# imaginateit/csm-train-pytorch

Measured on AMD Instinct MI355X. Metric: train tokens/sec (text+audio) CSM-1B bf16 seq2048, higher is better.
Workload: dtype bf16

## Files before the change

### csm-train-pytorch_amd/csm/engine.py

```python
from __future__ import annotations

from contextlib import contextmanager
from typing import Dict, List, Optional

import torch

from .hip import ops
from .sampling import (RowSampler, _is_number, check_filters, check_processors, check_row_processors,
                       check_sampling, names_processors)

BF16 = torch.bfloat16
F32 = torch.float32
import os as _os
FUSE_SWIGLU = _os.environ.get("CSM_FUSE_SWIGLU", "1") == "1"
FUSE_ROPE_BWD = _os.environ.get("CSM_FUSE_ROPE_BWD", "1") == "1"
FUSE_ROPE_FWD = _os.environ.get("CSM_FUSE_ROPE_FWD", "1") == "1"
PAIR_DX_DW = int(_os.environ.get("CSM_PAIR_DX_DW", "0"))
GROUP_ATTN_DW = _os.environ.get("CSM_GROUP_ATTN_DW", "1") == "1"
DEFER_ATTN_DW = int(_os.environ.get("CSM_DEFER_ATTN_DW", "3"))
DEFER_NORM_DW = _os.environ.get("CSM_DEFER_NORM_DW", "1") == "1"
ROWS_ON_HOST = _os.environ.get("CSM_ROWS_ON_HOST", "1") == "1"
EMB_KEYSORT = _os.environ.get("CSM_EMB_KEYSORT", "1") == "1"
DECODE_POS_HOST = _os.environ.get("CSM_DECODE_POS_HOST", "1") == "1"
LORA_FUSE = _os.environ.get("CSM_LORA_FUSE", "1") != "0"


def _refuse_stack(lo, where: str):
    if getattr(lo, "n_adapters", 1) > 1:
        raise ValueError(f"{where} takes one adapter set, and model.lora stacks {lo.n_adapters}: export one first "
                         "(state = model.lora.export(a), then LoRABank.add / generate_batch(adapters=[...]) / row_lora(model, state))")


def adapter_rows(adapter_ids, B: int, S: int, n_adapters: int, segment_lengths=None) -> torch.Tensor:
    ids = torch.as_tensor(adapter_ids).detach().to("cpu")
    if ids.is_floating_point() or ids.dtype == torch.bool:
        raise ValueError(f"adapter_ids must be integers, got {ids.dtype}")
    ids = ids.to(torch.int64)
    if segment_lengths is None:
        if tuple(ids.shape) != (B,):
            raise ValueError(f"adapter_ids must have shape [B={B}] (one adapter set per example), got {tuple(ids.shape)}")
        live = ids
        sel = ids.repeat_interleave(S)
    else:
        L = torch.as_tensor(segment_lengths).detach().to("cpu").to(torch.int64)
        if ids.dim() != 2 or tuple(ids.shape) != tuple(L.shape) or L.shape[0] != B:
            raise ValueError(f"adapter_ids of a packed batch must have the shape of segment_lengths {tuple(L.shape)} "
                             f"(one adapter set per segment), got {tuple(ids.shape)}")
        if bool((L < 0).any()) or bool((L.sum(1) > S).any()):
            raise ValueError("segment_lengths: negative, or more than a row holds")
        live = ids[L > 0]
        full_len = torch.cat([L, (S - L.sum(1))[:, None]], 1).reshape(-1)
        full_ids = torch.cat([ids, torch.full((B, 1), -1, dtype=torch.int64)], 1).reshape(-1)
        sel = torch.repeat_interleave(full_ids, full_len)
    if live.numel() and (int(live.min()) < -1 or int(live.max()) >= n_adapters):
        bad = live[(live < -1) | (live >= n_adapters)]
# ... 602 lines not shown
            ops.gemm(dl[0], ah[0], dxf[:, dd:2 * dd], None, False, False, batch=K - 1, sA=N * Vp, sB=dd * Vp, sC=dd)
            xf2 = dec["xf"].view(N, K * dd)
            if train_other:
                gah = m.block("audio_head.padded", True)
                ops.gemm(xf2[:, dd:2 * dd], dl[0], gah[0], gah[0] if acc["other"] else None, True, True, batch=K - 1, sA=dd,
                         sB=N * Vp, sC=dd * Vp, sR=dd * Vp)
            del dl
            dx0 = self.decoder.backward(dxf.view(N * K, dd), N, K, tr["decoder"], 1.0, on_layer_done=self.grad_hook,
                                        acc=acc["decoder"], sel=dec.get("sel"))
            dseq = torch.empty(N * K, d, dtype=BF16, device=dev)
            ops.linear_dx(dx0, m.block("projection.weight"), dseq)
            if train_other:
                ops.linear_dw(dx0, dec["seq"], m.block("projection.weight", True), accumulate=acc["other"])
            dec_pos0 = (dseq, dec["rows"], K)
            if self.grad_hook is not None:
                self.grad_hook("decoder", -1)

        dlog = torch.empty(M, Vp, dtype=BF16, device=dev)
        rows_loss = torch.empty(M, dtype=F32, device=dev)
        ops.ce_fwd_bwd(s["logits"], s["t0"], rows_loss, dlog, V, gscale * s["sw"] / s["n_sem"])
        dhid = torch.empty(M, d, dtype=BF16, device=dev)
        ops.linear_dx(dlog, m.block("codebook0_head.padded"), dhid)
        if train_other:
            ops.linear_dw(dlog, hidden, m.block("codebook0_head.padded", True), accumulate=acc["other"])
        del dlog
        if dec_pos0 is not None:
            ops.rows_add_bf16(dhid, dec_pos0[1], dec_pos0[0], dec_pos0[2])
        if self.grad_hook is not None:
            self.grad_hook("other", -1)

        dh0 = self.backbone.backward(dhid, B, S, tr["backbone"], 1.0, on_layer_done=self.grad_hook, acc=acc["backbone"], seg=s.get("seg"),
                                    sel=s.get("sel"))
        if train_embeddings:
            self._embedding_backward(s, dh0, dseq if (dec is not None and s["aw"] != 0.0) else None)
        if self.grad_hook is not None:
            self.grad_hook("embeddings", -1)

    def _embedding_backward(self, s, dh0, dseq):
        m, a = self.m, self.m.args
        dev = m.device
        K, V = a.audio_num_codebooks, a.audio_vocab_size
        TV = a.text_vocab_size
        n_rows = TV + K * V
        tk, mk = s["tk"], s["mk"]
        M = tk.shape[0]
        ck = ("embbwd", M, K, V, TV)
        c = self._consts.get(ck)
        if c is None:
            slot = torch.arange(K + 1, device=dev)
            c = self._consts[ck] = dict(off=torch.where(slot < K, TV + slot * V, torch.zeros_like(slot)),
                                        src=torch.arange(M, device=dev).unsqueeze(1).expand(M, K + 1).reshape(-1).contiguous())
        rows = torch.where(mk.bool(), tk + c["off"], torch.full_like(tk, n_rows)).reshape(-1)
        src = c["src"]
        n_src = M
        if dseq is not None:
            codes, N = s["dec"]["codes"], s["dec"]["N"]
            dk = ("embbwd_dec", M, N, K, V, TV)
            d = self._consts.get(dk)
            if d is None:
                d = self._consts[dk] = dict(off=TV + torch.arange(K - 1, device=dev) * V,
                                            src=(M + torch.arange(N, device=dev).unsqueeze(1) * K + torch.arange(1, K, device=dev)).reshape(-1))
            rows = torch.cat([rows, (codes[:, :K - 1] + d["off"]).reshape(-1)])
            src = torch.cat([src, d["src"]])
            n_src = M + N * K
        if n_src <= (1 << 20) and EMB_KEYSORT:
            key = torch.sort((rows << 20) | src).values
            rows_s, src_s = key >> 20, key & ((1 << 20) - 1)
        else:
            order = torch.argsort(rows, stable=True)
            rows_s, src_s = rows[order].contiguous(), src[order].contiguous()
        ops.embed_bwd_sorted(rows_s, src_s, dh0, dseq,
                             m.block("text_embeddings.weight", True), m.block("audio_embeddings.weight", True))

    @torch.no_grad()
    def hidden_states(self, tokens: torch.Tensor, masks: torch.Tensor) -> torch.Tensor:
        m, a = self.m, self.m.args
        B, S, K1 = tokens.shape
        M = B * S
        tk = tokens.reshape(M, K1).to(device=m.device, dtype=torch.int64).contiguous()
        mk = masks.reshape(M, K1).to(device=m.device, dtype=torch.uint8).contiguous()
        h0 = torch.empty(M, m.bb.embed_dim, dtype=BF16, device=m.device)
        self._need()
        ops.embed_fwd(tk, mk, m.block("text_embeddings.weight"), m.block("audio_embeddings.weight"), h0, a.audio_vocab_size)
        return self.backbone.forward(h0, B, S, False).view(B, S, -1)

    @torch.no_grad()
    def generate_frame(self, tokens, tokens_mask, input_pos, temperature, topk, noise=None, adapters=None, top_p=None,
                       min_p=None, repetition_penalty=None, repetition_window=None):
        m, a = self.m, self.m.args
        self._need()
        if int(input_pos[0, 0]) == 0:
            m._gen_adapters = list(adapters) if adapters is not None and any(x is not None for x in adapters) else None
        if not getattr(m, "use_kv_cache", True):
            if names_processors(temperature, topk, repetition_penalty=repetition_penalty, repetition_window=repetition_window):
                raise ValueError("the recompute path (use_kv_cache = False) has no repetition penalty and no per-codebook "
                                 "parameters: they need the KV-cache path")
            if top_p is not None or min_p is not None:
                raise ValueError("the recompute path (use_kv_cache = False) has no top_p / min_p: the filters need the KV-cache path")
            return self._generate_frame_recompute(tokens, tokens_mask, input_pos, temperature, topk, noise)
        dev = m.device
        K, V, Vp = a.audio_num_codebooks, a.audio_vocab_size, m.vocab_pad
        d, dd = m.bb.embed_dim, m.dc.embed_dim
        tokens, tokens_mask = tokens.to(dev), tokens_mask.to(dev)
        Bn, Sn, K1 = tokens.shape
        first = int(input_pos[0, 0]) == 0
# ... 688 lines not shown
```

### csm-train-pytorch_amd/csm/hip/__init__.py

```python
import ctypes as C
import os

_HERE = os.path.dirname(os.path.abspath(__file__))
LIB_PATH = os.environ.get("CSM_HIP_LIB") or os.path.join(_HERE, "libcsm_hip.so")


class CsmHipError(RuntimeError):
    pass


if not os.path.exists(LIB_PATH):
    raise ImportError(
        f"{LIB_PATH} is missing: build it with `python __graft_entry__.py build` (or `make -C csm-train-pytorch_amd/csrc`). "
        "The CSM MI355X path has no fallback implementation."
    )

lib = C.CDLL(LIB_PATH)

_p, _i, _f, _ll = C.c_void_p, C.c_int, C.c_float, C.c_longlong

_SIGS = {
    "csm_abi_version": ([], _i),
    "csm_last_error": ([], C.c_char_p),
    "csm_device_check": ([_i], _i),
# ... 5 lines not shown
    "csm_skinny_nt_bf16": ([_p, _p, _p, _i, _i, _i, _i, _i, _i, _f, _p], _i),
    "csm_skinny_nt_sel_bf16": ([_p, _p, _p, _p, _i, _i, _i, _i, _i, _i, _i, _f, _p], _i),
    "csm_gemm_bf16_dgrad_wgrad": ([_p, _p, _p, _p, _p, _i, _i, _i, _i, _i, _i, _i, _i, _i, _p, _i, _i, _f, _p], _i),
    "csm_gemm_bf16_two_wgrad": ([_p, _p, _p, _i, _i, _i, _i, _i, _p, _p, _p, _i, _i, _i, _i, _i, _i, _i, _f, _p], _i),
    "csm_gemm_bf16_multi_wgrad": ([_i, _p, _p, _p, _p, _p, _p, _p, _p, _i, _i, _f, _p], _i),
    "csm_set_gemm_variant": ([_i], _i),
    "csm_set_gemm256_persistent": ([_i], _i),
    "csm_get_gemm256_persistent": ([], _i),
    "csm_set_gemm_tuning": ([_i, _i], _i),
    "csm_gemm_last_kernel": ([], C.c_char_p),
    "csm_attn_bwd_workspace_bytes": ([_i, _i, _i], _ll),
    "csm_rmsnorm_fwd": ([_p, _p, _p, _p, _i, _i, _f, _p], _i),
    "csm_rmsnorm_bwd_blocks": ([], _i),
    "csm_rmsnorm_bwd": ([_p, _p, _p, _p, _p, _p, _p, _i, _i, _p], _i),
    "csm_colsum_bf16": ([_p, _i, _i, _p, _i, _p], _i),
    "csm_colsum_bf16_multi": ([_i, _p, _p, _i, _i, _i, _p], _i),
    "csm_dropout_bf16": ([_p, _i, _p, _i, _ll, _i, _f, C.c_ulonglong, _i, _p], _i),
    "csm_bias_add_bf16": ([_p, _i, _p, _ll, _i, _p], _i),
    "csm_colsum_rows_bf16": ([_p, _i, _ll, _i, _p, _i, _p], _i),
    "csm_rope": ([_p, _p, _p, _ll, _i, _i, _i, _i, _i, _p], _i),
    "csm_set_attn_variant": ([_i], _i),
    "csm_attn_last_dkv_kernel": ([], _i),
    "csm_attn64_set_debug": ([_p], _i),
    "csm_set_decode_tuning": ([_i, _i], _i),
    "csm_attn_fwd": ([_p, _p, _p, _i, _i, _i, _i, _i, _p], _i),
    "csm_attn_bwd": ([_p, _p, _p, _p, _p, _p, _i, _i, _i, _i, _i, _p], _i),
    "csm_attn_bwd_rope": ([_p, _p, _p, _p, _p, _p, _p, _i, _i, _i, _i, _i, _p], _i),
    "csm_attn_fwd_seg": ([_p, _p, _p, _p, _i, _i, _i, _i, _i, _p], _i),
    "csm_attn_bwd_seg": ([_p, _p, _p, _p, _p, _p, _p, _p, _i, _i, _i, _i, _i, _p], _i),
    "csm_swiglu_fwd": ([_p, _p, _ll, _i, _p], _i),
    "csm_swiglu_bwd": ([_p, _p, _p, _ll, _i, _p], _i),
    "csm_embed_fwd": ([_p, _p, _p, _p, _p, _ll, _i, _i, _i, _p], _i),
    "csm_embed_bwd_sorted": ([_p, _p, _ll, _p, _p, _ll, _p, _p, _ll, _ll, _i, _p], _i),
    "csm_rows_add_bf16": ([_p, _p, _p, _ll, _i, _i, _p], _i),
    "csm_rows_take_bf16": ([_p, _p, _p, _ll, _i, _p], _i),
    "csm_decoder_input_fwd": ([_p, _p, _p, _p, _p, _ll, _i, _i, _i, _p], _i),
    "csm_ce_fwd_bwd": ([_p, _p, _p, _p, _ll, _i, _i, _i, _f, _p], _i),
    "csm_reduce_sum_f32": ([_p, _ll, _f, _p, _p], _i),
    "csm_sumsq_blocks": ([], _i),
    "csm_sumsq_bf16": ([_p, _ll, _p, _p], _i),
    "csm_clip_coef": ([_p, _i, _f, _p, _p], _i),
    "csm_adamw_step": ([_p, _p, _p, _p, _p, _ll, _f, _f, _f, _f, _f, _i, _p, _f, _i, _p], _i),
    "csm_adamw_step_split": ([_p, _p, _p, _p, _p, _ll, _f, _f, _f, _f, _f, _i, _p, _f, _i, _p], _i),
    "csm_adamw_step_live": ([_p, _p, _p, _p, _p, _ll, _f, _f, _f, _f, _f, _i, _p, _f, _i, _p, _p], _i),
    "csm_adamw_step_split_live": ([_p, _p, _p, _p, _p, _ll, _f, _f, _f, _f, _f, _i, _p, _f, _i, _p, _p], _i),
    "csm_set_adamw_blocks": ([_i], _i),
    "csm_gemv_bf16": ([_p, _p, _p, _p, _i, _i, _i, _i, _i, _i, _i, _p], _i),
    "csm_gemv_last_kernel": ([], C.c_char_p),
    "csm_gemv_bf16_kext": ([_p, _p, _p, _p, _i, _i, _i, _i, _i, _i, _i, _p, _f, _i, _p, _i, _p, _p, _i, _i, _i, _p, _p], _i),
    "csm_lora_project_bf16": ([_p, _p, _p, _i, _i, _i, _i, _i, _i, _f, _p, _f, _p], _i),
    "csm_lora_project_rows_bf16": ([_p, _p, _p, _p, _p, _i, _i, _i, _i, _i, _i, _i, _p, _f, _p], _i),
    "csm_gemv_bf16_kext_rows": ([_p, _p, _p, _p, _i, _i, _i, _i, _i, _i, _i, _p, _f, _i, _p, _i, _p, _p, _p, _p, _i, _i, _i, _i, _p], _i),
    "csm_gemv_t_bf16": ([_p, _p, _p, _i, _i, _i, _i, _i, _i, _i, _p], _i),
    "csm_gemv_bf16_ex": ([_p, _p, _p, _p, _i, _i, _i, _i, _i, _i, _i, _p, _f, _i, _p, _i, _p], _i),
    "csm_quantize_rows_fp8": ([_p, _p, _p, _i, _i, _i, _i, _p], _i),
    "csm_gemv_fp8w": ([_p, _p, _p, _p, _p, _i, _i, _i, _i, _i, _i, _i, _p, _f, _i, _p, _i, _p], _i),
    "csm_gemv_fp8w_kext_rows": ([_p, _p, _p, _p, _p, _i, _i, _i, _i, _i, _i, _i, _p, _f, _i, _p, _i, _p, _p, _p, _p, _i, _i, _i, _i, _p], _i),
    "csm_attn_decode_rope": ([_p, _p, _p, _p, _p, _p, _i, _i, _i, _i, _i, _i, _p], _i),
    "csm_gemv_attn_bf16": ([_p, _p, _p, _p, _p, _p, _p, _p, _i, _i, _i, _i, _i, _i, _i, _i, _i, _p], _i),
    "csm_gemv_attn_at_bf16": ([_p, _p, _p, _i, _p, _p, _p, _p, _i, _i, _i, _i, _i, _i, _p], _i),
    "csm_attn_decode_rope_at": ([_p, _p, _p, _p, _i, _p, _i, _i, _i, _i, _i, _i, _p], _i),
    "csm_attn_append": ([_p, _p, _p, _p, _i, _i, _i, _i, _i, _i, _i, _f, _p], _i),
    "csm_attn_append_rows": ([_p, _p, _p, _p, _p, _p, _p, _i, _i, _i, _i, _i, _f, _p], _i),
    "csm_kv_append": ([_p, _p, _p, _p, _i, _i, _i, _i, _i, _i, _p], _i),
    "csm_kv_shift": ([_p, _p, _p, _i, _i, _i, _i, _i, _i, _i, _p], _i),
    "csm_attn_decode": ([_p, _p, _p, _p, _p, _i, _i, _i, _i, _i, _i, _p], _i),
# ... 65 lines not shown
```

### csm-train-pytorch_amd/csm/hip/ops.py

```python
import ctypes
import math
from typing import Optional

import torch

from . import CsmHipError, check, lib

BF16 = torch.bfloat16


def _stream() -> int:
    return torch.cuda.current_stream().cuda_stream


def _ptr(t: Optional[torch.Tensor]) -> Optional[int]:
    return None if t is None else t.data_ptr()


def _mat(t: torch.Tensor, dtype=BF16):
    assert t.is_cuda and t.dtype == dtype and t.dim() == 2 and t.stride(1) == 1, (t.dtype, t.shape, t.stride())
    return t.data_ptr(), t.shape[0], t.shape[1], t.stride(0)


def _pin(pin):
# ... 283 lines not shown
    assert delta_ws.dtype == torch.float32 and delta_ws.is_contiguous() and delta_ws.numel() * 4 >= need, f"delta_ws: {need} bytes of scratch"
    check(lib.csm_attn_bwd_seg(qkv.data_ptr(), out.data_ptr(), dout.data_ptr(), lse.data_ptr(), dqkv.data_ptr(), delta_ws.data_ptr(),
                               _seg_array(seg_start, B, S), _seg_array(seg_end, B, S), B, S, H, KV, HD, _stream()), "csm_attn_bwd_seg")
    return dqkv


def swiglu_fwd(gu, out):
    M, F2 = gu.shape
    check(lib.csm_swiglu_fwd(gu.data_ptr(), out.data_ptr(), M, F2 // 2, _stream()), "csm_swiglu_fwd")
    return out


def swiglu_bwd(gu, dout, dgu):
    M, F2 = gu.shape
    check(lib.csm_swiglu_bwd(gu.data_ptr(), dout.data_ptr(), dgu.data_ptr(), M, F2 // 2, _stream()), "csm_swiglu_bwd")
    return dgu


def embed_fwd(tokens, mask_u8, text_emb, audio_emb, out, audio_vocab):
    M, K1 = tokens.shape
    assert tokens.dtype == torch.int64 and mask_u8.dtype == torch.uint8 and tokens.is_contiguous() and mask_u8.is_contiguous()
    check(lib.csm_embed_fwd(tokens.data_ptr(), mask_u8.data_ptr(), text_emb.data_ptr(), audio_emb.data_ptr(), out.data_ptr(),
                            M, K1 - 1, out.shape[1], audio_vocab, _stream()), "csm_embed_fwd")
    return out


def embed_bwd_sorted(sorted_rows, src_index, dh, dseq, g_text, g_audio):
    assert sorted_rows.dtype == torch.int64 and src_index.dtype == torch.int64 and sorted_rows.is_contiguous() and src_index.is_contiguous()
    check(lib.csm_embed_bwd_sorted(sorted_rows.data_ptr(), src_index.data_ptr(), sorted_rows.numel(), dh.data_ptr(), _ptr(dseq),
                                   dh.shape[0], g_text.data_ptr(), g_audio.data_ptr(), g_text.shape[0],
                                   g_text.shape[0] + g_audio.shape[0], dh.shape[1], _stream()), "csm_embed_bwd_sorted")


def rows_add_bf16(dst, rows_i32, src, src_stride_rows):
    check(lib.csm_rows_add_bf16(dst.data_ptr(), rows_i32.data_ptr(), src.data_ptr(), rows_i32.numel(), int(src_stride_rows),
                                dst.shape[1], _stream()), "csm_rows_add_bf16")


def rows_take_bf16(table, rows_i32, out):
    assert rows_i32.dtype == torch.int32 and rows_i32.is_contiguous() and out.is_contiguous() and out.shape == (rows_i32.numel(), table.shape[1])
    check(lib.csm_rows_take_bf16(table.data_ptr(), rows_i32.data_ptr(), out.data_ptr(), rows_i32.numel(), table.shape[1], _stream()),
          "csm_rows_take_bf16")
    return out


def decoder_input_fwd(hidden, rows_i32, codes, audio_emb, out, audio_vocab):
    N, K = codes.shape
    assert rows_i32.dtype == torch.int32 and codes.dtype == torch.int64 and codes.is_contiguous()
    check(lib.csm_decoder_input_fwd(hidden.data_ptr(), rows_i32.data_ptr(), codes.data_ptr(), audio_emb.data_ptr(),
                                    out.data_ptr(), N, K, hidden.shape[1], audio_vocab, _stream()), "csm_decoder_input_fwd")
    return out


def ce_fwd_bwd(logits_f32, targets, loss_rows, dlogits, V, grad_scale):
    R, ldl = logits_f32.shape[0], logits_f32.stride(0)
    assert logits_f32.dtype == torch.float32 and targets.dtype == torch.int64 and targets.is_contiguous()
    ldd = dlogits.stride(0) if dlogits is not None else 0
    check(lib.csm_ce_fwd_bwd(logits_f32.data_ptr(), targets.data_ptr(), loss_rows.data_ptr(), _ptr(dlogits), R, V, ldl, ldd,
                             float(grad_scale), _stream()), "csm_ce_fwd_bwd")


def reduce_sum(x_f32, out_f32, scale=1.0):
    check(lib.csm_reduce_sum_f32(x_f32.data_ptr(), x_f32.numel(), float(scale), out_f32.data_ptr(), _stream()), "csm_reduce_sum_f32")


def sumsq_blocks() -> int:
# ... 514 lines not shown
```

### csm-train-pytorch_amd/csrc/ops.hip

```cpp
#include "common.h"
#include <math.h>

namespace {

template <int NC>
__global__ __launch_bounds__(256) void rmsnorm_fwd_kernel(const bf16_t* __restrict__ x, const bf16_t* __restrict__ w,
                                                          bf16_t* __restrict__ y, float* __restrict__ rstd, int M, int D,
                                                          float eps) {
    const int lane = threadIdx.x & 63;
    const int wpb = blockDim.x >> 6;
    const int nchunk = D >> 3;
    for (long long row = (long long)blockIdx.x * wpb + (threadIdx.x >> 6); row < M; row += (long long)gridDim.x * wpb) {
        U4 v[NC];
        float ss = 0.f;
#pragma unroll
        for (int i = 0; i < NC; ++i) {
            const int c = lane + 64 * i;
            v[i] = (U4){0u, 0u, 0u, 0u};
            if (c < nchunk) v[i] = *reinterpret_cast<const U4*>(x + (size_t)row * D + c * 8);
            float f[8];
            unpack8(v[i], f);
#pragma unroll
            for (int j = 0; j < 8; ++j) ss += f[j] * f[j];
        }
        ss = wave_sum(ss);
        const float r = rsqrtf(ss / (float)D + eps);
        if (lane == 0 && rstd) rstd[row] = r;
#pragma unroll
        for (int i = 0; i < NC; ++i) {
            const int c = lane + 64 * i;
            if (c < nchunk) {
                float f[8], s[8];
                unpack8(v[i], f);
                unpack8(*reinterpret_cast<const U4*>(w + c * 8), s);
// ... 302 lines not shown
#pragma unroll
    for (int c = 0; c < NC; ++c)
#pragma unroll
        for (int j = 0; j < 8; ++j) acc[c][j] = 0.f;
    const int nchunk = D >> 3;
    for (long long k = i; k < n_occ && rows[k] == r; ++k) {
        const long long sidx = src[k];
        const bf16_t* p = sidx < M ? dh + (size_t)sidx * D : dseq + (size_t)(sidx - M) * D;
#pragma unroll
        for (int c = 0; c < NC; ++c) {
            const int ch = lane + 64 * c;
            if (ch < nchunk) {
                float f[8];
                unpack8(*reinterpret_cast<const U4*>(p + ch * 8), f);
#pragma unroll
                for (int j = 0; j < 8; ++j) acc[c][j] += f[j];
            }
        }
    }
    bf16_t* dst = r < text_rows ? g_text + (size_t)r * D : g_audio + (size_t)(r - text_rows) * D;
#pragma unroll
    for (int c = 0; c < NC; ++c) {
        const int ch = lane + 64 * c;
        if (ch < nchunk) {
            float f[8];
            unpack8(*reinterpret_cast<const U4*>(dst + ch * 8), f);
#pragma unroll
            for (int j = 0; j < 8; ++j) f[j] += acc[c][j];
            *reinterpret_cast<U4*>(dst + ch * 8) = pack8(f);
        }
    }
}

__global__ __launch_bounds__(256) void rows_add_kernel(bf16_t* __restrict__ dst, const int* __restrict__ rows,
                                                       const bf16_t* __restrict__ src, long long N, int src_stride_rows, int D) {
    const int lane = threadIdx.x & 63;
    const long long n = (long long)blockIdx.x * (blockDim.x >> 6) + (threadIdx.x >> 6);
    if (n >= N) return;
    if (rows[n] < 0) return;
    bf16_t* d = dst + (size_t)rows[n] * D;
    const bf16_t* s = src + (size_t)n * src_stride_rows * D;
    for (int c0 = lane * 8; c0 < D; c0 += 512) {
        float a[8], b[8];
        unpack8(*reinterpret_cast<const U4*>(d + c0), a);
        unpack8(*reinterpret_cast<const U4*>(s + c0), b);
#pragma unroll
        for (int j = 0; j < 8; ++j) a[j] += b[j];
        *reinterpret_cast<U4*>(d + c0) = pack8(a);
    }
}

__global__ __launch_bounds__(256) void rows_take_kernel(bf16_t* __restrict__ table, const int* __restrict__ rows,
                                                        bf16_t* __restrict__ out, long long N, int D) {
    const int lane = threadIdx.x & 63;
    const long long n = (long long)blockIdx.x * (blockDim.x >> 6) + (threadIdx.x >> 6);
    if (n >= N) return;
    const int r = rows[n];
    bf16_t* o = out + (size_t)n * D;
    const U4 z = {0u, 0u, 0u, 0u};
    for (int c0 = lane * 8; c0 < D; c0 += 512) {
        if (r < 0) { *reinterpret_cast<U4*>(o + c0) = z; continue; }
        bf16_t* t = table + (size_t)r * D + c0;
        *reinterpret_cast<U4*>(o + c0) = *reinterpret_cast<const U4*>(t);
        *reinterpret_cast<U4*>(t) = z;
    }
}
// ... 515 lines not shown
                "csm_decoder_input_fwd: bad arguments");
    hipLaunchKernelGGL(decoder_input_kernel, dim3((unsigned)(N * K)), dim3(256), 0, stream, (const bf16_t*)hidden, rows, codes,
                       (const bf16_t*)audio_emb, (bf16_t*)out, K, D, audio_vocab);
    CSM_CHECK_LAUNCH("csm_decoder_input_fwd");
    return 0;
}

extern "C" int csm_ce_fwd_bwd(const float* logits, const long long* targets, float* loss_rows, void* dlogits, long long R,
                              int V, int ldl, int ldd, float grad_scale, hipStream_t stream) {
    CSM_REQUIRE(logits && targets && loss_rows && R > 0 && R < (1ll << 31) && V > 0 && ldl >= V, "csm_ce_fwd_bwd: bad arguments");
    CSM_REQUIRE(!dlogits || ldd >= V, "csm_ce_fwd_bwd: ldd < V");
    const int width = ldl > ldd && dlogits ? ldl : (dlogits ? ldd : ldl);
    const bool vec = (ldl & 3) == 0 && ((uintptr_t)logits & 15) == 0 && (!dlogits || ((ldd & 3) == 0 && ((uintptr_t)dlogits & 7) == 0 && ldd <= ldl + 0));
    if (vec && width <= 256 * 12) {
        const dim3 grid((unsigned)((R + 3) / 4)), block(256);
#define L(NC) hipLaunchKernelGGL((ce_wave_kernel<NC>), grid, block, 0, stream, logits, targets, loss_rows, (bf16_t*)dlogits, R, V, ldl, ldd, grad_scale)
        if (width <= 256 * 4) L(4); else if (width <= 256 * 9) L(9); else L(12);
#undef L
    } else {
        hipLaunchKernelGGL(ce_kernel, dim3((unsigned)R), dim3(256), 0, stream, logits, targets, loss_rows, (bf16_t*)dlogits, V, ldl,
                           ldd, grad_scale);
    }
    CSM_CHECK_LAUNCH("csm_ce_fwd_bwd");
    return 0;
}

extern "C" int csm_reduce_sum_f32(const float* x, long long n, float scale, float* out, hipStream_t stream) {
    CSM_REQUIRE(x && out && n > 0, "csm_reduce_sum_f32: bad arguments");
    hipLaunchKernelGGL(reduce_sum_kernel, dim3(1), dim3(1024), 0, stream, x, n, scale, out);
    CSM_CHECK_LAUNCH("csm_reduce_sum_f32");
    return 0;
}

#define CSM_SUMSQ_BLOCKS 8192
extern "C" int csm_sumsq_blocks(void) { return CSM_SUMSQ_BLOCKS; }

extern "C" int csm_sumsq_bf16(const void* g, long long n, float* partials, hipStream_t stream) {
    CSM_REQUIRE(g && partials && n > 0 && ((uintptr_t)g & 15) == 0, "csm_sumsq_bf16: bad arguments");
    hipLaunchKernelGGL(sumsq_kernel, dim3(CSM_SUMSQ_BLOCKS), dim3(256), 0, stream, (const bf16_t*)g, n, partials);
    CSM_CHECK_LAUNCH("csm_sumsq_bf16");
    return 0;
}

extern "C" int csm_clip_coef(const float* partials, int n_partials, float max_norm, float* norm_and_coef,
                             hipStream_t stream) {
    CSM_REQUIRE(partials && norm_and_coef && n_partials > 0, "csm_clip_coef: bad arguments");
    hipLaunchKernelGGL(clip_coef_kernel, dim3(1), dim3(1024), 0, stream, partials, n_partials, max_norm, norm_and_coef);
    CSM_CHECK_LAUNCH("csm_clip_coef");
    return 0;
}

static int g_adamw_blocks = 1 << 20;
extern "C" int csm_set_adamw_blocks(int b) { g_adamw_blocks = b; return 0; }

extern "C" int csm_adamw_step(float* master, float* m, float* v, void* param, void* grad, long long n, float lr,
                              float beta1, float beta2, float eps, float weight_decay, int step,
                              const float* norm_and_coef, float grad_mul, int zero_grad, hipStream_t stream) {
    CSM_REQUIRE(master && m && v && param && grad && n > 0 && step > 0, "csm_adamw_step: bad arguments");
    CSM_REQUIRE((n & 7) == 0, "csm_adamw_step: n must be a multiple of 8 (pad the arena)");
    const float bc1 = 1.f - powf(beta1, (float)step);
    const float bc2s = sqrtf(1.f - powf(beta2, (float)step));
    hipLaunchKernelGGL(adamw_kernel, dim3(grid_for(n >> 3, 256, g_adamw_blocks)), dim3(256), 0, stream, master, m, v, (bf16_t*)param,
                       (bf16_t*)grad, n, lr, beta1, beta2, eps, weight_decay, bc1, bc2s, norm_and_coef, grad_mul, zero_grad);
    CSM_CHECK_LAUNCH("csm_adamw_step");
    return 0;
}
// ... 43 lines not shown
```

### include/csm_hip.h

```cpp
#ifndef CSM_HIP_H
#define CSM_HIP_H
#include <stdint.h>

#ifdef __cplusplus
extern "C" {
#endif

typedef struct ihipStream_t* csm_stream_t;

int csm_abi_version(void);
const char* csm_last_error(void);
int csm_device_check(int device);

int csm_gemm_bf16(const void* A, const void* B, void* C, const void* R, int M, int N, int K, int lda, int ldb, int ldc,
                  int ldr, int transA, int transB, int out_f32, float alpha, int batch, long long strideA,
                  long long strideB, long long strideC, long long strideR, csm_stream_t stream);

int csm_gemm_bf16_ex(const void* A, const void* B, void* C, const void* R, int M, int N, int K, int lda, int ldb, int ldc,
                     int ldr, int transA, int transB, int out_f32, float alpha, int batch, long long strideA,
                     long long strideB, long long strideC, long long strideR, int epilogue, const void* aux_in,
                     void* aux_out, int ld_aux, csm_stream_t stream);
int csm_gemm_bf16_rope(const void* A, const void* W, void* C, int M, int N, int K, int lda, int ldw, int ldc,
                       const float* rope_table, int rows_per_seq, int n_rope_cols, int head_dim, csm_stream_t stream);
int csm_gemm_bf16_kext(const void* A, const void* B, void* C, const void* R, int M, int N, int K, int lda, int ldb, int ldc, int ldr,
// ... 31 lines not shown
int csm_colsum_bf16_multi(int n, const float* const* partials, void* const* dst, int rows, int D, int accumulate, csm_stream_t stream);

int csm_dropout_bf16(const void* in, int ld_in, void* out, int ld_out, long long M, int D, float p, unsigned long long seed,
                     int accumulate, csm_stream_t stream);
int csm_bias_add_bf16(void* y, int ld, const void* bias, long long M, int D, csm_stream_t stream);
int csm_colsum_rows_bf16(const void* x, int ld, long long M, int D, float* partials , int slices,
                         csm_stream_t stream);

int csm_rope(void* qkv, const float* table, const int* pos, long long M, int S, int n_heads_qk, int head_dim, int ld,
             int inverse, csm_stream_t stream);

int csm_set_attn_variant(int v);
int csm_attn_fwd(const void* qkv, void* out, float* lse, int B, int S, int H, int KV, int HD, csm_stream_t stream);
long long csm_attn_bwd_workspace_bytes(int B, int S, int H);
int csm_attn_bwd(const void* qkv, const void* out, const void* dout, const float* lse, void* dqkv,
                 float* delta_ws , int B, int S, int H, int KV, int HD, csm_stream_t stream);
int csm_attn_bwd_rope(const void* qkv, const void* out, const void* dout, const float* lse, void* dqkv, float* delta_ws,
                      const float* rope_table, int B, int S, int H, int KV, int HD, csm_stream_t stream);
int csm_attn_last_dkv_kernel(void);
int csm_attn_fwd_seg(const void* qkv, void* out, float* lse, const int* seg_start, int B, int S, int H, int KV, int HD, csm_stream_t stream);
int csm_attn_bwd_seg(const void* qkv, const void* out, const void* dout, const float* lse, void* dqkv, float* delta_ws,
                     const int* seg_start, const int* seg_end, int B, int S, int H, int KV, int HD, csm_stream_t stream);
int csm_attn64_set_debug(void* device_buffer);

int csm_swiglu_fwd(const void* gu, void* out, long long M, int F, csm_stream_t stream);
int csm_swiglu_bwd(const void* gu, const void* dout, void* dgu, long long M, int F, csm_stream_t stream);

int csm_embed_fwd(const long long* tokens, const uint8_t* mask, const void* text_emb, const void* audio_emb, void* out,
                  long long M, int K, int D, int audio_vocab, csm_stream_t stream);

int csm_embed_bwd_sorted(const long long* sorted_rows, const long long* src_index, long long n_occ, const void* dh,
                         const void* dseq, long long M, void* g_text, void* g_audio, long long text_rows, long long n_rows,
                         int D, csm_stream_t stream);
int csm_rows_add_bf16(void* dst, const int* rows, const void* src, long long N, int src_stride_rows, int D, csm_stream_t stream);
int csm_rows_take_bf16(void* table, const int* rows, void* out, long long N, int D, csm_stream_t stream);

int csm_decoder_input_fwd(const void* hidden, const int* rows, const long long* codes, const void* audio_emb, void* out,
                          long long N, int K, int D, int audio_vocab, csm_stream_t stream);

int csm_ce_fwd_bwd(const float* logits, const long long* targets, float* loss_rows, void* dlogits, long long R, int V,
                   int ldl, int ldd, float grad_scale, csm_stream_t stream);
int csm_reduce_sum_f32(const float* x, long long n, float scale, float* out, csm_stream_t stream);

int csm_sumsq_blocks(void);
int csm_sumsq_bf16(const void* g, long long n, float* partials , csm_stream_t stream);
int csm_clip_coef(const float* partials, int n_partials, float max_norm, float* norm_and_coef , csm_stream_t stream);
int csm_adamw_step(float* master, float* m, float* v, void* param, void* grad, long long n, float lr, float beta1,
                   float beta2, float eps, float weight_decay, int step, const float* norm_and_coef ,
                   float grad_mul, int zero_grad , csm_stream_t stream);
int csm_adamw_step_split(void* master_lo, float* m, float* v, void* param, void* grad, long long n, float lr, float beta1,
                         float beta2, float eps, float weight_decay, int step, const float* norm_and_coef, float grad_mul,
                         int zero_grad, csm_stream_t stream);
int csm_adamw_step_live(float* master, float* m, float* v, void* param, void* grad, long long n, float lr, float beta1,
                        float beta2, float eps, float weight_decay, int step, const float* norm_and_coef, float grad_mul,
                        int zero_grad, void* block_live, csm_stream_t stream);
int csm_adamw_step_split_live(void* master_lo, float* m, float* v, void* param, void* grad, long long n, float lr, float beta1,
                              float beta2, float eps, float weight_decay, int step, const float* norm_and_coef, float grad_mul,
                              int zero_grad, void* block_live, csm_stream_t stream);

int csm_set_adamw_blocks(int blocks);

int csm_sample_topk(const float* logits, const float* q, int* out, int rows, int V, int ldl, int topk, float temperature,
                    csm_stream_t stream);
int csm_sample_topk_rows(const float* logits, const float* q, int* out, int rows, int V, int ldl, const int* topk,
                         const float* temperature, csm_stream_t stream);
int csm_sample_filtered_rows(const float* logits, const float* q, int* out, int rows, int V, int ldl, const int* topk,
                             const float* temperature, const float* top_p, const float* min_p, csm_stream_t stream);
#define CSM_SAMPLE_HIST 64
int csm_sample_processed_rows(const float* logits, const float* q, int* out, int rows, int V, int ldl, const int* topk,
                              const float* temperature, const float* top_p, const float* min_p, const float* penalty,
                              const int* window, int* hist, int ldh, int* frame, const int* live, int advance,
                              csm_stream_t stream);

int csm_set_decode_tuning(int key, int value);
int csm_gemv_bf16(const void* x, const void* W, void* y, const void* residual, int B, int N, int K, int ldw, int ldx, int ldy,
                  int out_f32, csm_stream_t stream);
// ... 101 lines not shown
```

Before: 127,200.

## Build embedding-backward sort index with per-column block radix sort and run-segmented scatter

Replaces the torch-built row/src listing and global torch.sort in the embedding backward with a custom HIP kernel that radix-sorts each codebook column in one block and emits concatenated sorted rows and sources plus a device-side count. A new run-based accumulation kernel has each wavefront find runs of equal rows in a chunk, sum their gradients in fp32, and write each row once. When the table gradient is known to be zero it skips reading the old values. This removes several small torch launches and the generic sort, at the cost of size limits (M+N at most 9216, vocab at most 2^17) and a fallback path for larger inputs.

```diff
diff --git a/csm-train-pytorch_amd/csm/engine.py b/csm-train-pytorch_amd/csm/engine.py
--- a/csm-train-pytorch_amd/csm/engine.py
+++ b/csm-train-pytorch_amd/csm/engine.py
@@ -21,6 +21,8 @@
 DEFER_NORM_DW = _os.environ.get("CSM_DEFER_NORM_DW", "1") == "1"
 ROWS_ON_HOST = _os.environ.get("CSM_ROWS_ON_HOST", "1") == "1"
 EMB_KEYSORT = _os.environ.get("CSM_EMB_KEYSORT", "1") == "1"
+EMB_INDEX = _os.environ.get("CSM_EMB_INDEX", "1") == "1"
+EMB_RUNS = _os.environ.get("CSM_EMB_RUNS", "1") == "1"
 DECODE_POS_HOST = _os.environ.get("CSM_DECODE_POS_HOST", "1") == "1"
 LORA_FUSE = _os.environ.get("CSM_LORA_FUSE", "1") != "0"
 
@@ -689,11 +691,12 @@
         dh0 = self.backbone.backward(dhid, B, S, tr["backbone"], 1.0, on_layer_done=self.grad_hook, acc=acc["backbone"], seg=s.get("seg"),
                                     sel=s.get("sel"))
         if train_embeddings:
-            self._embedding_backward(s, dh0, dseq if (dec is not None and s["aw"] != 0.0) else None)
+            table_zero = not acc["embeddings"] and self.grad_hook is None
+            self._embedding_backward(s, dh0, dseq if (dec is not None and s["aw"] != 0.0) else None, table_zero)
         if self.grad_hook is not None:
             self.grad_hook("embeddings", -1)
 
-    def _embedding_backward(self, s, dh0, dseq):
+    def _embedding_backward(self, s, dh0, dseq, table_zero=False):
         m, a = self.m, self.m.args
         dev = m.device
         K, V = a.audio_num_codebooks, a.audio_vocab_size
@@ -701,6 +704,16 @@
         n_rows = TV + K * V
         tk, mk = s["tk"], s["mk"]
         M = tk.shape[0]
+        g_text, g_audio = m.block("text_embeddings.weight", True), m.block("audio_embeddings.weight", True)
+        codes = s["dec"]["codes"] if dseq is not None else None
+        if EMB_INDEX and ops.embed_bwd_index_supported(M, 0 if codes is None else codes.shape[0], K, V, TV):
+            rows_s, src_s, n_occ = ops.embed_bwd_index(tk, mk, codes, V, TV)
+            if EMB_RUNS:
+                ops.embed_bwd_runs(rows_s, src_s, dh0, dseq, g_text, g_audio, n_occ=n_occ, table_zero=table_zero)
+            else:
+                live = torch.arange(rows_s.numel(), device=dev) < n_occ
+                ops.embed_bwd_sorted(torch.where(live, rows_s, n_rows), torch.where(live, src_s, 0), dh0, dseq, g_text, g_audio)
+            return
         ck = ("embbwd", M, K, V, TV)
         c = self._consts.get(ck)
         if c is None:
@@ -726,8 +739,10 @@
         else:
             order = torch.argsort(rows, stable=True)
             rows_s, src_s = rows[order].contiguous(), src[order].contiguous()
-        ops.embed_bwd_sorted(rows_s, src_s, dh0, dseq,
-                             m.block("text_embeddings.weight", True), m.block("audio_embeddings.weight", True))
+        if EMB_RUNS:
+            ops.embed_bwd_runs(rows_s, src_s, dh0, dseq, g_text, g_audio, table_zero=table_zero)
+        else:
+            ops.embed_bwd_sorted(rows_s, src_s, dh0, dseq, g_text, g_audio)
 
     @torch.no_grad()
     def hidden_states(self, tokens: torch.Tensor, masks: torch.Tensor) -> torch.Tensor:
diff --git a/csm-train-pytorch_amd/csm/hip/__init__.py b/csm-train-pytorch_amd/csm/hip/__init__.py
--- a/csm-train-pytorch_amd/csm/hip/__init__.py
+++ b/csm-train-pytorch_amd/csm/hip/__init__.py
@@ -61,6 +61,10 @@
     "csm_swiglu_bwd": ([_p, _p, _p, _ll, _i, _p], _i),
     "csm_embed_fwd": ([_p, _p, _p, _p, _p, _ll, _i, _i, _i, _p], _i),
     "csm_embed_bwd_sorted": ([_p, _p, _ll, _p, _p, _ll, _p, _p, _ll, _ll, _i, _p], _i),
+    "csm_embed_bwd_runs": ([_p, _p, _ll, _p, _p, _p, _ll, _p, _p, _ll, _ll, _i, _i, _p], _i),
+    "csm_embed_bwd_index_supported": ([_ll, _ll, _i, _i, _i], _i),
+    "csm_embed_bwd_index_workspace": ([_i], _ll),
+    "csm_embed_bwd_index": ([_p, _p, _p, _ll, _ll, _i, _i, _i, _p, _p, _p, _p, _p], _i),
     "csm_rows_add_bf16": ([_p, _p, _p, _ll, _i, _i, _p], _i),
     "csm_rows_take_bf16": ([_p, _p, _p, _ll, _i, _p], _i),
     "csm_decoder_input_fwd": ([_p, _p, _p, _p, _p, _ll, _i, _i, _i, _p], _i),
diff --git a/csm-train-pytorch_amd/csm/hip/ops.py b/csm-train-pytorch_amd/csm/hip/ops.py
--- a/csm-train-pytorch_amd/csm/hip/ops.py
+++ b/csm-train-pytorch_amd/csm/hip/ops.py
@@ -339,6 +339,34 @@
                                    g_text.shape[0] + g_audio.shape[0], dh.shape[1], _stream()), "csm_embed_bwd_sorted")
 
 
+def embed_bwd_runs(sorted_rows, src_index, dh, dseq, g_text, g_audio, n_occ=None, table_zero=False):
+    assert sorted_rows.dtype == torch.int64 and src_index.dtype == torch.int64 and sorted_rows.is_contiguous() and src_index.is_contiguous()
+    assert n_occ is None or (n_occ.dtype == torch.int64 and n_occ.numel() == 1)
+    check(lib.csm_embed_bwd_runs(sorted_rows.data_ptr(), src_index.data_ptr(), sorted_rows.numel(), _ptr(n_occ), dh.data_ptr(),
+                                 _ptr(dseq), dh.shape[0], g_text.data_ptr(), g_audio.data_ptr(), g_text.shape[0],
+                                 g_text.shape[0] + g_audio.shape[0], dh.shape[1], int(bool(table_zero)), _stream()), "csm_embed_bwd_runs")
+
+
+def embed_bwd_index_supported(M, N, K, V, TV) -> bool:
+    return bool(lib.csm_embed_bwd_index_supported(M, N, K, V, TV))
+
+
+def embed_bwd_index(tokens, mask_u8, codes, V, TV):
+    M, K1 = tokens.shape
+    K = K1 - 1
+    N = 0 if codes is None else codes.shape[0]
+    assert tokens.dtype == torch.int64 and mask_u8.dtype == torch.uint8 and tokens.is_contiguous() and mask_u8.is_contiguous()
+    assert codes is None or (codes.dtype == torch.int64 and codes.is_contiguous() and codes.shape[1] == K)
+    cap = M * K1 + N * (K - 1)
+    rows_s = torch.empty(cap, dtype=torch.int64, device=tokens.device)
+    src_s = torch.empty(cap, dtype=torch.int64, device=tokens.device)
+    n_occ = torch.empty(1, dtype=torch.int64, device=tokens.device)
+    ws = torch.empty(lib.csm_embed_bwd_index_workspace(K), dtype=torch.uint8, device=tokens.device)
+    check(lib.csm_embed_bwd_index(tokens.data_ptr(), mask_u8.data_ptr(), _ptr(codes) if N else None, M, N, K, V, TV, rows_s.data_ptr(),
+                                  src_s.data_ptr(), n_occ.data_ptr(), ws.data_ptr(), _stream()), "csm_embed_bwd_index")
+    return rows_s, src_s, n_occ
+
+
 def rows_add_bf16(dst, rows_i32, src, src_stride_rows):
     check(lib.csm_rows_add_bf16(dst.data_ptr(), rows_i32.data_ptr(), src.data_ptr(), rows_i32.numel(), int(src_stride_rows),
                                 dst.shape[1], _stream()), "csm_rows_add_bf16")
diff --git a/csm-train-pytorch_amd/csrc/ops.hip b/csm-train-pytorch_amd/csrc/ops.hip
--- a/csm-train-pytorch_amd/csrc/ops.hip
+++ b/csm-train-pytorch_amd/csrc/ops.hip
@@ -1,5 +1,6 @@
 #include "common.h"
 #include <math.h>
+#include <rocprim/block/block_radix_sort.hpp>
 
 namespace {
 
@@ -368,6 +369,172 @@
     }
 }
 
+constexpr int EBR_CHUNK = 16, EBR_DEPTH = 2;
+__device__ __forceinline__ long long readlane_ll(long long v, int l) {
+    const unsigned lo = (unsigned)__builtin_amdgcn_readlane((int)(unsigned)(unsigned long long)v, l);
+    const unsigned hi = (unsigned)__builtin_amdgcn_readlane((int)(unsigned)((unsigned long long)v >> 32), l);
+    return (long long)(((unsigned long long)hi << 32) | lo);
+}
+
+template <int NC>
+__global__ __launch_bounds__(256) void embed_bwd_runs_kernel(const long long* __restrict__ rows, const long long* __restrict__ src,
+                                                             long long n_cap, const long long* __restrict__ n_dev,
+                                                             const bf16_t* __restrict__ dh, const bf16_t* __restrict__ dseq, long long M,
+                                                             bf16_t* __restrict__ g_text, bf16_t* __restrict__ g_audio,
+                                                             long long text_rows, long long n_rows, int D, int table_zero) {
+    constexpr int chunk = EBR_CHUNK, DEPTH = EBR_DEPTH;
+    const int lane = threadIdx.x & 63;
+    const long long base = ((long long)blockIdx.x * (blockDim.x >> 6) + (threadIdx.x >> 6)) * chunk;
+    long long n = n_cap;
+    if (n_dev) { const long long nd = *n_dev; n = nd < n_cap ? nd : n_cap; }
+    if (base >= n) return;
+    const long long pos = base + lane;
+    long long r = n_rows, rp = -1, s = 0;
+    if (lane < chunk && pos < n) {
+        r = rows[pos];
+        s = src[pos];
+        if (pos > 0) rp = rows[pos - 1];
+    }
+    unsigned long long heads = __ballot(r >= 0 && r < n_rows && r != rp);
+    const int nchunk = D >> 3;
+    while (heads) {
+        const int h = __builtin_amdgcn_readfirstlane(__ffsll(heads) - 1);
+        heads &= heads - 1;
+        const long long rh = readlane_ll(r, h);
+        const int e = h + __popcll(__ballot(r == rh));
+        float acc[NC][8];
+#pragma unroll
+        for (int c = 0; c < NC; ++c)
+#pragma unroll
+            for (int j = 0; j < 8; ++j) acc[c][j] = 0.f;
+        bf16_t* dst = rh < text_rows ? g_text + (size_t)rh * D : g_audio + (size_t)(rh - text_rows) * D;
+        U4 dq[NC];
+#pragma unroll
+        for (int c = 0; c < NC; ++c) {
+            dq[c] = (U4){0u, 0u, 0u, 0u};
+            if (!table_zero && lane + 64 * c < nchunk) dq[c] = *reinterpret_cast<const U4*>(dst + (lane + 64 * c) * 8);
+        }
+        for (int k = h; k < e; k += DEPTH) {
+            U4 q[DEPTH][NC];
+#pragma unroll
+            for (int u = 0; u < DEPTH; ++u) {
+                if (k + u < e) {
+                    const long long sidx = readlane_ll(s, k + u);
+                    const bf16_t* p = sidx < M ? dh + (size_t)sidx * D : dseq + (size_t)(sidx - M) * D;
+#pragma unroll
+                    for (int c = 0; c < NC; ++c) {
+                        const int ch = lane + 64 * c;
+                        if (ch < nchunk) q[u][c] = *reinterpret_cast<const U4*>(p + ch * 8);
+                    }
+                }
+            }
+#pragma unroll
+            for (int u = 0; u < DEPTH; ++u) {
+                if (k + u < e) {
+#pragma unroll
+                    for (int c = 0; c < NC; ++c) {
+                        const int ch = lane + 64 * c;
+                        if (ch < nchunk) {
+                            float f[8];
+                            unpack8(q[u][c], f);
+#pragma unroll
+                            for (int j = 0; j < 8; ++j) acc[c][j] += f[j];
+                        }
+                    }
+                }
+            }
+        }
+        if (e == chunk) {
+            for (long long k = base + chunk; k < n && rows[k] == rh; ++k) {
+                const long long sidx = src[k];
+                const bf16_t* p = sidx < M ? dh + (size_t)sidx * D : dseq + (size_t)(sidx - M) * D;
+#pragma unroll
+                for (int c = 0; c < NC; ++c) {
+                    const int ch = lane + 64 * c;
+                    if (ch < nchunk) {
+                        float f[8];
+                        unpack8(*reinterpret_cast<const U4*>(p + ch * 8), f);
+#pragma unroll
+                        for (int j = 0; j < 8; ++j) acc[c][j] += f[j];
+                    }
+                }
+            }
+        }
+#pragma unroll
+        for (int c = 0; c < NC; ++c) {
+            const int ch = lane + 64 * c;
+            if (ch < nchunk) {
+                float f[8];
+                unpack8(dq[c], f);
+#pragma unroll
+                for (int j = 0; j < 8; ++j) f[j] += acc[c][j];
+                *reinterpret_cast<U4*>(dst + ch * 8) = pack8(f);
+            }
+        }
+    }
+}
+
+constexpr int EIX_THREADS = 1024, EIX_ITEMS = 9, EIX_CAP = EIX_THREADS * EIX_ITEMS, EIX_IDX_BITS = 14, EIX_MAX_VOCAB = 1 << 17;
+static_assert(EIX_CAP <= (1 << EIX_IDX_BITS), "the listing index must fit its key bits");
+using EixSort = rocprim::block_radix_sort<unsigned int, EIX_THREADS, EIX_ITEMS>;
+
+__global__ __launch_bounds__(EIX_THREADS) void embed_bwd_index_sort_kernel(const long long* __restrict__ tokens, const uint8_t* __restrict__ masks,
+                                                                           const long long* __restrict__ codes, int M, int N, int K,
+                                                                           int V, int TV, unsigned* __restrict__ keys_ws,
+                                                                           int* __restrict__ counts) {
+    __shared__ typename EixSort::storage_type storage;
+    __shared__ int live_total;
+    const int col = blockIdx.x == 0 ? K : (int)blockIdx.x - 1;
+    const long long vocab = col == K ? TV : V;
+    const int n_in = M + ((codes && col < K - 1) ? N : 0);
+    if (threadIdx.x == 0) live_total = 0;
+    __syncthreads();
+    unsigned key[EIX_ITEMS];
+    int live = 0;
+#pragma unroll
+    for (int j = 0; j < EIX_ITEMS; ++j) {
+        const int idx = threadIdx.x * EIX_ITEMS + j;
+        key[j] = 0xffffffffu;
+        long long tok = -1;
+        if (idx < M) {
+            if (masks[(size_t)idx * (K + 1) + col]) tok = tokens[(size_t)idx * (K + 1) + col];
+        } else if (idx < n_in) {
+            tok = codes[(size_t)(idx - M) * K + col];
+        }
+        if (tok >= 0 && tok < vocab) {
+            key[j] = ((unsigned)tok << EIX_IDX_BITS) | (unsigned)idx;
+            ++live;
+        }
+    }
+    if (live) atomicAdd(&live_total, live);
+    int id_bits = 1;
+    while ((1ll << id_bits) <= vocab) ++id_bits;
+    EixSort().sort(key, storage, EIX_IDX_BITS, EIX_IDX_BITS + id_bits);
+    unsigned* out = keys_ws + (size_t)blockIdx.x * EIX_CAP + threadIdx.x * EIX_ITEMS;
+#pragma unroll
+    for (int j = 0; j < EIX_ITEMS; ++j) out[j] = key[j];
+    __syncthreads();
+    if (threadIdx.x == 0) counts[blockIdx.x] = live_total;
+}
+
+__global__ __launch_bounds__(256) void embed_bwd_index_emit_kernel(const unsigned* __restrict__ keys_ws, const int* __restrict__ counts,
+                                                                   int M, int K, int V, int TV, long long* __restrict__ rows_s,
+                                                                   long long* __restrict__ src_s, long long* __restrict__ n_occ) {
+    const int slot = blockIdx.y;
+    const int col = slot == 0 ? K : slot - 1;
+    long long off = 0;
+    for (int i = 0; i < slot; ++i) off += counts[i];
+    const int cnt = counts[slot];
+    if (slot == (int)gridDim.y - 1 && blockIdx.x == 0 && threadIdx.x == 0) n_occ[0] = off + cnt;
+    const long long rowbase = col == K ? 0 : (long long)TV + (long long)col * V;
+    for (int p = blockIdx.x * blockDim.x + threadIdx.x; p < cnt; p += gridDim.x * blockDim.x) {
+        const unsigned key = keys_ws[(size_t)slot * EIX_CAP + p];
+        const long long idx = key & ((1u << EIX_IDX_BITS) - 1);
+        rows_s[off + p] = rowbase + (key >> EIX_IDX_BITS);
+        src_s[off + p] = idx < M ? idx : M + (idx - M) * K + col + 1;
+    }
+}
+
 __global__ __launch_bounds__(256) void rows_add_kernel(bf16_t* __restrict__ dst, const int* __restrict__ rows,
                                                        const bf16_t* __restrict__ src, long long N, int src_stride_rows, int D) {
     const int lane = threadIdx.x & 63;
@@ -949,6 +1116,45 @@
     return 0;
 }
 
+extern "C" int csm_embed_bwd_index_supported(long long M, long long N, int K, int V, int TV) {
+    return M > 0 && N >= 0 && M + N <= EIX_CAP && K >= 1 && K < 65535 && V > 0 && V <= EIX_MAX_VOCAB && TV > 0 && TV <= EIX_MAX_VOCAB;
+}
+
+extern "C" long long csm_embed_bwd_index_workspace(int K) { return ((long long)(K + 1) * EIX_CAP + (K + 1)) * 4; }
+
+extern "C" int csm_embed_bwd_index(const long long* tokens, const uint8_t* masks, const long long* codes, long long M, long long N,
+                                   int K, int V, int TV, long long* rows_s, long long* src_s, long long* n_occ, void* workspace,
+                                   hipStream_t stream) {
+    CSM_REQUIRE(tokens && masks && rows_s && src_s && n_occ && workspace && (codes || N == 0), "csm_embed_bwd_index: bad arguments");
+    CSM_REQUIRE(csm_embed_bwd_index_supported(M, N, K, V, TV),
+                "csm_embed_bwd_index: M + N = %lld (<= %d), K = %d, V = %d, TV = %d (<= %d) is outside the kernel's limits", M + N, EIX_CAP,
+                K, V, TV, EIX_MAX_VOCAB);
+    unsigned* keys_ws = (unsigned*)workspace;
+    int* counts = (int*)(keys_ws + (size_t)(K + 1) * EIX_CAP);
+    hipLaunchKernelGGL(embed_bwd_index_sort_kernel, dim3(K + 1), dim3(EIX_THREADS), 0, stream, tokens, masks, N > 0 ? codes : nullptr,
+                       (int)M, (int)N, K, V, TV, keys_ws, counts);
+    CSM_CHECK_LAUNCH("csm_embed_bwd_index (sort)");
+    hipLaunchKernelGGL(embed_bwd_index_emit_kernel, dim3(EIX_CAP / 256, K + 1), dim3(256), 0, stream, keys_ws, counts, (int)M, K, V, TV,
+                       rows_s, src_s, n_occ);
+    CSM_CHECK_LAUNCH("csm_embed_bwd_index (emit)");
+    return 0;
+}
+
+extern "C" int csm_embed_bwd_runs(const long long* sorted_rows, const long long* src_index, long long n_cap, const long long* n_occ_dev,
+                                  const void* dh, const void* dseq, long long M, void* g_text, void* g_audio, long long text_rows,
+                                  long long n_rows, int D, int table_zero, hipStream_t stream) {
+    CSM_REQUIRE(sorted_rows && src_index && dh && g_text && g_audio && n_cap > 0, "csm_embed_bwd_runs: bad arguments");
+    CSM_REQUIRE((D & 7) == 0 && D <= 4096, "csm_embed_bwd_runs: D=%d must be a multiple of 8 and <= 4096", D);
+    const long long blocks = (n_cap + 4 * EBR_CHUNK - 1) / (4 * EBR_CHUNK);
+    CSM_REQUIRE(blocks < (1ll << 31), "csm_embed_bwd_runs: too many occurrences");
+    const int nchunk = D / 8;
+#define L(NC) hipLaunchKernelGGL((embed_bwd_runs_kernel<NC>), dim3((unsigned)blocks), dim3(256), 0, stream, sorted_rows, src_index, n_cap, n_occ_dev, (const bf16_t*)dh, (const bf16_t*)dseq, M, (bf16_t*)g_text, (bf16_t*)g_audio, text_rows, n_rows, D, table_zero)
+    if (nchunk <= 64) L(1); else if (nchunk <= 128) L(2); else if (nchunk <= 256) L(4); else L(8);
+#undef L
+    CSM_CHECK_LAUNCH("csm_embed_bwd_runs");
+    return 0;
+}
+
 #define CSM_SUMSQ_BLOCKS 8192
 extern "C" int csm_sumsq_blocks(void) { return CSM_SUMSQ_BLOCKS; }
 
diff --git a/include/csm_hip.h b/include/csm_hip.h
--- a/include/csm_hip.h
+++ b/include/csm_hip.h
@@ -87,6 +87,13 @@
 int csm_embed_bwd_sorted(const long long* sorted_rows, const long long* src_index, long long n_occ, const void* dh,
                          const void* dseq, long long M, void* g_text, void* g_audio, long long text_rows, long long n_rows,
                          int D, csm_stream_t stream);
+int csm_embed_bwd_runs(const long long* sorted_rows, const long long* src_index, long long n_cap, const long long* n_occ_dev,
+                       const void* dh, const void* dseq, long long M, void* g_text, void* g_audio, long long text_rows,
+                       long long n_rows, int D, int table_zero, csm_stream_t stream);
+int csm_embed_bwd_index_supported(long long M, long long N, int K, int V, int TV);
+long long csm_embed_bwd_index_workspace(int K);
+int csm_embed_bwd_index(const long long* tokens, const uint8_t* masks, const long long* codes, long long M, long long N, int K, int V,
+                        int TV, long long* rows_s, long long* src_s, long long* n_occ, void* workspace, csm_stream_t stream);
 int csm_rows_add_bf16(void* dst, const int* rows, const void* src, long long N, int src_stride_rows, int D, csm_stream_t stream);
 int csm_rows_take_bf16(void* table, const int* rows, void* out, long long N, int D, csm_stream_t stream);
 
@@ -96,7 +103,6 @@
 int csm_ce_fwd_bwd(const float* logits, const long long* targets, float* loss_rows, void* dlogits, long long R, int V,
                    int ldl, int ldd, float grad_scale, csm_stream_t stream);
 int csm_reduce_sum_f32(const float* x, long long n, float scale, float* out, csm_stream_t stream);
-
 int csm_sumsq_blocks(void);
 int csm_sumsq_bf16(const void* g, long long n, float* partials , csm_stream_t stream);
 int csm_clip_coef(const float* partials, int n_partials, float max_norm, float* norm_and_coef , csm_stream_t stream);
```

New measurement: 128,200 (median of 6 runs). No clear change (+0.8%).
